# LivGen/LMAT

Measured on AMD Instinct MI355X. Metric: reads/s (150 bp) vs 64 GB k-mer DB, higher is better.
Workload: dtype u64; 1 GPU; 1104000000 x 150 bp reads/GPU vs 64 GiB k-mer hash (6467472668 20-mers, replicated per GPU), run_rl.sh flags -x 0 -j 30 -l 0 -b 1, calls-only; total_reads=1104000000, reads_per_launch=8000000, read_len=150, db_kmers=6467472668, k=20, parallelism=reads sharded x1, DB replicated, genus_block_permille=100, prune_g=0, list_replicas=1, distinct_lists=792576, reads_called=1058323347, read_pool_batches=32

## Files before the change

include/lmat_hip.h:

```cpp
#ifndef LMAT_HIP_H
#define LMAT_HIP_H

#include <stddef.h>
#include <stdint.h>

#ifdef __cplusplus
extern "C" {
#endif

#define LMAT_OK 0
#define LMAT_E_ARG (-1)
#define LMAT_E_IO (-2)
#define LMAT_E_DEVICE (-3)
#define LMAT_E_CAPACITY (-4)
#define LMAT_E_TAXONOMY (-5)
#define LMAT_E_NOMEM (-6)
#define LMAT_E_STATE (-7)
#define LMAT_E_INTERNAL (-8)

typedef struct lmat_ctx lmat_ctx;
typedef struct lmat_reads lmat_reads;
typedef struct lmat_ingest lmat_ingest;
typedef struct lmat_stream lmat_stream;

// ... 219 lines not shown
    uint64_t reads, bases;
    uint64_t windows;
    uint64_t runs;
    uint32_t passes;
    uint32_t prefix_bits;
    float extract_ms, sort_ms, segment_ms, histogram_ms;
} lmat_cov_stats;
int lmat_cov_create(lmat_ctx* ctx, const int* k_sizes, int n_k, lmat_cov** out);
void lmat_cov_destroy(lmat_cov* c);
const char* lmat_cov_error(const lmat_cov* c);
int lmat_cov_set_options(lmat_cov* c, uint64_t device_budget_bytes , int prefix_bits );
int lmat_cov_add_reads(lmat_cov* c, const uint8_t* ascii, const uint64_t* off , uint64_t n_reads, const uint32_t* group);
int lmat_cov_run(lmat_cov* c, lmat_cov_stats* out);
int lmat_cov_summary(lmat_cov* c, int k_index, uint32_t* groups, uint64_t* distinct, uint64_t* total, uint64_t cap, uint64_t* n);
int lmat_cov_histogram(lmat_cov* c, int k_index, uint32_t group, uint64_t* multiplicity, uint64_t* n_kmers, uint64_t cap, uint64_t* n);

int lmat_debug_decide(lmat_ctx* ctx, const uint32_t* tids, const float* scores, const uint64_t* off, const float* stdev,
                      uint64_t n, lmat_read_result* results);
int lmat_debug_decide_counts(lmat_ctx* ctx, const uint32_t* tids, const uint32_t* counts, const uint64_t* off, const uint32_t* cand,
                             uint64_t n, int on_the_wave, lmat_read_result* results);
int lmat_debug_decide_chain(lmat_ctx* ctx, const uint32_t* tids, const uint32_t* counts, const uint64_t* off, const uint32_t* cand,
                            const uint32_t* kept, const uint32_t* eligible, uint64_t n, int with_cands, lmat_read_result* results,
                            uint8_t* took);

int lmat_gather_bench(lmat_ctx* ctx, uint64_t n_probes, uint64_t seed, float* ms, uint64_t* bytes);

int lmat_table_address(int k, uint64_t want_buckets, uint64_t kmer, uint64_t* n_buckets, uint32_t* bucket, uint32_t* tag);
int lmat_table_unaddress(int k, uint64_t want_buckets, uint32_t bucket, uint32_t tag, uint64_t* kmer);

int64_t lmat_format_out(const lmat_ctx* ctx, const lmat_read_result* results, uint64_t n, const lmat_cand* cands,
                        const uint8_t* bases, const uint64_t* off, int prn_read, uint64_t first_index, char* buf,
                        uint64_t cap);

#ifdef __cplusplus
}
#endif
#endif
```

lmat_amd/capi.py:

```python
from __future__ import annotations

import ctypes as C
import os

import numpy as np

_HERE = os.path.dirname(os.path.abspath(__file__))
LIB_PATH = os.environ.get("LMAT_LIB") or os.path.join(_HERE, "liblmat_hip.so")


class LmatError(RuntimeError):
    def __init__(self, code, msg):
        super().__init__(f"lmat error {code}: {msg}")
        self.code = code


class Params(C.Structure):
    _fields_ = [("sdiff", C.c_float), ("hbias", C.c_float), ("min_score", C.c_float), ("min_kmer", C.c_int32),
                ("min_fnd_kmer", C.c_int32), ("prn_all", C.c_int32), ("screen_phix", C.c_int32)]

    @classmethod
    def run_rl(cls, prn_all=1):
        return cls(1.0, 0.0, 0.0, 30, 1, prn_all, 1)

# ... 116 lines not shown
        "lmat_counts_get": (i32, [vp, vp, vp, vp, u32, P(u32), vp]),
        "lmat_gather_bench": (i32, [vp, u64, u64, P(C.c_float), P(u64)]),
        "lmat_stream_create": (i32, [vp, u64, u64, u32, i32, P(vp)]),
        "lmat_stream_acquire": (i32, [vp, P(vp), P(vp)]),
        "lmat_stream_submit": (i32, [vp, u64, u64]),
        "lmat_stream_submit_from": (i32, [vp, vp, vp, u64, u64]),
        "lmat_host_alloc": (i32, [u64, P(vp)]),
        "lmat_host_free": (None, [vp]),
        "lmat_stream_next": (i32, [vp, P(vp), P(vp), P(u64), P(u64), P(u64)]),
        "lmat_stream_release": (i32, [vp]),
        "lmat_stream_destroy": (None, [vp]),
        "lmat_debug_stream_stats": (i32, [vp, vp]),
        "lmat_debug_reads_words": (i32, [vp, vp, u64, u64, vp, vp]),
        "lmat_counts_allreduce": (i32, [P(vp), i32]),
        "lmat_comm_unique_id": (i32, [vp]),
        "lmat_comm_init": (i32, [vp, vp, i32, i32]),
        "lmat_comm_allreduce_counts": (i32, [vp]),
        "lmat_comm_size": (i32, [vp]),
        "lmat_comm_destroy": (None, [vp]),
        "lmat_db_clone": (i32, [vp, vp]),
        "lmat_debug_decide": (i32, [vp, vp, vp, vp, vp, u64, vp]),
        "lmat_debug_decide_counts": (i32, [vp, vp, vp, vp, vp, u64, i32, vp]),
        "lmat_debug_decide_chain": (i32, [vp, vp, vp, vp, vp, vp, vp, u64, i32, vp, vp]),
        "lmat_synth_window": (i32, [vp, u32, u64, P(u64), vp, u32, P(u32)]),
        "lmat_debug_last_counters": (i32, [vp, vp]),
        "lmat_debug_probe_stats": (i32, [vp, vp, u64, vp]),
        "lmat_debug_div_check": (i32, [vp, vp]),
        "lmat_debug_variant_launches": (i32, [vp, vp]),
        "lmat_debug_uniform_launches": (i32, [vp, vp]),
        "lmat_synth_read_windows": (i32, [vp, vp, u32, u64, u64, vp, vp, vp, u32, u32, P(u32), P(u32)]),
        "lmat_table_address": (i32, [i32, u64, u64, P(u64), P(u32), P(u32)]),
        "lmat_format_out": (C.c_int64, [vp, vp, u64, vp, vp, vp, i32, u64, vp, u64]),
        "lmat_build_create": (i32, [vp, i32, cp, P(vp)]),
        "lmat_build_destroy": (None, [vp]),
        "lmat_build_error": (cp, [vp]),
        "lmat_build_set_options": (i32, [vp, u64, i32, u32]),
        "lmat_build_add_fasta": (i32, [vp, cp]),
        "lmat_build_add_sequence": (i32, [vp, u32, vp, u64]),
        "lmat_build_run": (i32, [vp, P(BuildStats)]),
        "lmat_build_write_taxhisto": (i32, [vp, cp]),
        "lmat_build_fetch": (i32, [vp, u64, u64, vp, vp, vp, u64]),
        "lmat_db_build_from_genomes": (i32, [vp, vp, u64]),
        "lmat_build_add_taxhisto": (i32, [vp, cp]),
        "lmat_build_merge_stats": (i32, [vp, P(MergeStats)]),
        "lmat_build_taxid_counts": (i32, [vp, vp, vp, u64, P(u64)]),
        "lmat_cov_create": (i32, [vp, vp, i32, P(vp)]),
# ... 17 lines not shown
        "lmat_table_unaddress": (i32, [i32, u64, u32, u32, P(u64)]),
    }
    for name, (res, args) in sig.items():
        fn = getattr(lib, name)
        fn.restype = res
        fn.argtypes = args
    if path is None:
        _lib = lib
    return lib


EXPORTED = ["lmat_device_count", "lmat_ctx_create", "lmat_ctx_destroy", "lmat_last_error", "lmat_set_params", "lmat_taxonomy_load_files",
            "lmat_db_begin", "lmat_genedb_begin", "lmat_db_add_taxhisto", "lmat_db_finalize", "lmat_db_kmer_length", "lmat_db_size", "lmat_db_list_count", "lmat_db_arena_bytes",
            "lmat_db_set_build_options", "lmat_db_save_image", "lmat_db_load_image", "lmat_ingest_create", "lmat_ingest_idmap_from_tree", "lmat_rand_mode", "lmat_rand_reset", "lmat_rand_label", "lmat_rand_get",
            "lmat_ingest_destroy", "lmat_ingest_error", "lmat_ingest_set_options", "lmat_ingest_add_taxhisto",
            "lmat_ingest_save_image", "lmat_ingest_load_image", "lmat_ingest_size", "lmat_ingest_kmer_length",
            "lmat_ingest_lookup", "lmat_db_from_ingest", "lmat_nullmodel_load", "lmat_nullmodel_clear", "lmat_set_label_modes",
            "lmat_db_table_bytes", "lmat_db_lookup", "lmat_synth_taxonomy", "lmat_synth_db_build", "lmat_synth_db_build2", "lmat_synth_db_build3", "lmat_reads_upload",
            "lmat_reads_synth", "lmat_reads_download_ascii", "lmat_reads_count", "lmat_reads_device_bytes",
            "lmat_reads_free", "lmat_classify", "lmat_classify_async", "lmat_classify_async_cands", "lmat_comm_available", "lmat_sync", "lmat_last_timing", "lmat_results_fetch",
            "lmat_counts_reset", "lmat_counts_layout", "lmat_counts_device_ptr", "lmat_counts_get", "lmat_gather_bench",
            "lmat_table_address", "lmat_format_out", "lmat_stream_create", "lmat_stream_acquire", "lmat_stream_submit", "lmat_stream_submit_from", "lmat_host_alloc", "lmat_host_free",
            "lmat_stream_next", "lmat_stream_release", "lmat_stream_destroy", "lmat_counts_allreduce",
            "lmat_comm_unique_id", "lmat_comm_init", "lmat_comm_allreduce_counts", "lmat_comm_size", "lmat_comm_destroy", "lmat_db_clone", "lmat_debug_decide", "lmat_debug_decide_counts", "lmat_debug_decide_chain", "lmat_synth_window", "lmat_synth_read_windows", "lmat_debug_probe_stats", "lmat_debug_last_counters", "lmat_debug_div_check", "lmat_debug_variant_launches", "lmat_debug_uniform_launches",
            "lmat_build_create", "lmat_build_destroy", "lmat_build_error", "lmat_build_set_options", "lmat_build_add_fasta", "lmat_build_add_sequence",
            "lmat_build_run", "lmat_build_write_taxhisto", "lmat_build_fetch", "lmat_db_build_from_genomes",
            "lmat_build_add_taxhisto", "lmat_build_merge_stats", "lmat_build_taxid_counts",
            "lmat_cov_create", "lmat_cov_destroy", "lmat_cov_error", "lmat_cov_set_options", "lmat_cov_add_reads", "lmat_cov_run",
            "lmat_cov_summary", "lmat_cov_histogram",
            "lmat_export_create", "lmat_export_destroy", "lmat_export_error", "lmat_export_set_options", "lmat_export_run", "lmat_export_fetch",
            "lmat_export_taxid_counts", "lmat_build_add_db", "lmat_table_unaddress",
            "lmat_genebuild_create", "lmat_genedb_build_from_genes",
            "lmat_debug_stream_stats", "lmat_debug_reads_words"]


def _ptr(a):
    return a.ctypes.data_as(C.c_void_p) if a is not None else None


class Reads:
    def __init__(self, eng, handle):
        self.eng, self.h = eng, handle

    def __len__(self):
        return int(self.eng.lib.lmat_reads_count(self.h))

    @property
# ... 699 lines not shown
    def debug_decide_counts(self, tids, counts, off, cand, on_the_wave):
        tids = np.ascontiguousarray(tids, dtype=np.uint32)
        counts = np.ascontiguousarray(counts, dtype=np.uint32)
        off = np.ascontiguousarray(off, dtype=np.uint64)
        cand = np.ascontiguousarray(cand, dtype=np.uint32)
        res = np.zeros(cand.size, dtype=READ_RESULT_DTYPE)
        self._chk(self.lib.lmat_debug_decide_counts(self.ctx, _ptr(tids), _ptr(counts), _ptr(off), _ptr(cand), cand.size, int(on_the_wave), _ptr(res)))
        return res

    def debug_decide_chain(self, tids, counts, off, cand, kept, eligible, with_cands=False):
        tids = np.ascontiguousarray(tids, dtype=np.uint32)
        counts = np.ascontiguousarray(counts, dtype=np.uint32)
        off = np.ascontiguousarray(off, dtype=np.uint64)
        cand = np.ascontiguousarray(cand, dtype=np.uint32)
        kept = np.ascontiguousarray(kept, dtype=np.uint32)
        eligible = np.ascontiguousarray(eligible, dtype=np.uint32)
        assert kept.size == cand.size and eligible.size == cand.size and off.size == cand.size + 1
        res = np.zeros(cand.size, dtype=READ_RESULT_DTYPE)
        took = np.zeros(cand.size, dtype=np.uint8)
        self._chk(self.lib.lmat_debug_decide_chain(self.ctx, _ptr(tids), _ptr(counts), _ptr(off), _ptr(cand), _ptr(kept), _ptr(eligible),
                                                   cand.size, int(with_cands), _ptr(res), _ptr(took)))
        return res, took

    def clone_db_from(self, src: "Engine"):
        self._chk(self.lib.lmat_db_clone(self.ctx, src.ctx))

    def counts(self):
        n, _ = self.counts_layout()
        tid = np.zeros(n, dtype=np.uint32)
        cnt = np.zeros(n, dtype=np.uint64)
        sc = np.zeros(n, dtype=np.float64)
        nz = C.c_uint32(0)
        nm = np.zeros(3, dtype=np.uint64)
        self._chk(self.lib.lmat_counts_get(self.ctx, _ptr(tid), _ptr(cnt), _ptr(sc), n, C.byref(nz), _ptr(nm)))
        k = int(nz.value)
        return {int(t): (int(c), float(s)) for t, c, s in zip(tid[:k], cnt[:k], sc[:k])}, [int(x) for x in nm]
```

lmat_amd/csrc/kernels.hip:

```cpp
#include <hip/hip_runtime.h>
#include <atomic>
#include <type_traits>
#include "kernels.hpp"

#ifndef LMAT_ABLATE
#define LMAT_ABLATE 0
#endif
#define STOP_AT(n, v) do { if (LMAT_ABLATE && A.prm.stop_after == (n)) { if (lane == 0) { emit(250, (v)); } return; } } while (0)
#ifndef LMAT_CLOSURE_FAST
#define LMAT_CLOSURE_FAST 1
#endif
#ifndef LMAT_LDS_SHIFT
#define LMAT_LDS_SHIFT 0
#endif

namespace lmat {

#define WSYNC()                                              \
    do {                                                     \
        __builtin_amdgcn_fence(__ATOMIC_SEQ_CST, "wavefront"); \
        __builtin_amdgcn_wave_barrier();                     \
    } while (0)

template <bool GMEM>
// ... 939 lines not shown
    }
    if (bad) atomicAdd(out + 2, (unsigned long long)bad);
    atomicAdd(out + 3, 64ull);
}
typedef const ClassifyArgs __attribute__((address_space(4))) CArgsK4;
typedef float f32x4 __attribute__((ext_vector_type(4)));
__device__ __forceinline__ uint64_t bal(bool b) { return __builtin_amdgcn_ballot_w64(b); }
__device__ __forceinline__ void k4_wave_record(CArgsK4* Ap, int lane, GAS uint64_t* out, const lmat_read_result& res, uint32_t call_idx) {
    if (lane == 0) {
        GAS unsigned long long* tally_count = (GAS unsigned long long*)Ap->counts;
        GAS double* tally_score = (GAS double*)(tally_count + Ap->tb.n_ids);
        GAS unsigned long long* tally_nomatch = (GAS unsigned long long*)(tally_score + Ap->tb.n_ids);
        store_result(out, res);
        if (res.status != LMAT_ST_PHIX && res.match_type == LMAT_MT_NOMATCH) {
            G_ADD(&tally_nomatch[1], 1ull);
        } else if (res.call_score >= Ap->prm.min_score) {
            G_ADD(&tally_count[call_idx], 1ull);
            G_ADD(&tally_score[call_idx], (double)res.call_score);
        } else if (res.call_score < Ap->prm.min_score) {
            G_ADD(&tally_nomatch[2], 1ull);
        }
    }
}
__device__ __forceinline__ bool k4_wave_chain(CArgsK4* Ap, int lane, uint32_t nT, uint32_t cand, const u32x4 fz, uint32_t my_cnt,
                                              uint32_t my_id, uint32_t dep, uint32_t fl, uint32_t chain, uint32_t* xch, GAS uint64_t* out,
                                              int valid_kmers, uint32_t len, int bin_sel) {
    const uint32_t sx0 = chain & 63u, nK = (chain >> 8) & 0x7Fu;
    if (nK - 1u >= nT - 1u || sx0 >= nK) return false;
    const uint64_t am = below_mask_1_64((int)nT), KEPT = below_mask_1_64((int)nK), CH = am & ~KEPT, OTH = KEPT & ~(1ull << sx0);
    const uint32_t ti = fz.z & 0xFFFFu, oi = fz.z >> 16;
    const uint32_t c0 = rl(my_cnt, (int)sx0), riv = rl(fz.z, (int)sx0);
    const uint32_t rt = riv & 0xFFFFu, ro = riv >> 16;
    const uint32_t badfl = (uint32_t)kFlagPlasmid | (Ap->prm.screen_phix ? (uint32_t)kFlagPhiX : 0u);
    if ((~bal(my_cnt < c0) & OTH) | (~bal(my_cnt == c0) & CH)) return false;
    if ((~(bal(oi < rt) | bal(ro < ti)) & OTH) | (~(bal(ti < rt) & bal(ro <= oi)) & CH)) return false;
    if (!(bal(dep == 0u) & CH) || bal((fl & badfl) != 0)) return false;
    float* xs = (float*)xch;
    float* xv = (float*)(xch + 256);
    const float sc = div_small_ints((float)my_cnt, (float)cand);
    xs[lane] = sc;
    WSYNC();
    float log_sum = 0.0f;
    for (uint32_t t = 0; t < nT; t += 4) {
        const u32x4 q = *(const u32x4*)((const uint32_t*)xs + t);
        log_sum += __uint_as_float(q.x); log_sum += __uint_as_float(q.y); log_sum += __uint_as_float(q.z); log_sum += __uint_as_float(q.w);
    }
    const uint32_t pos_sig_hits = (uint32_t)popc64(bal(my_cnt > 0));
    const uint32_t use_sig_hits = pos_sig_hits > 3 ? pos_sig_hits : nT;
    const float log_avg = div_small_ints(log_sum, (float)use_sig_hits);
    const float dv = log_avg - sc;
    xv[lane] = (uint32_t)lane < nT && (pos_sig_hits > 3 ? my_cnt > 0 : true) ? dv * dv : 0.0f;
    WSYNC();
    float log_std = 0.0f;
    for (uint32_t t = 0; t < nT; t += 4) {
        const f32x4 q = *(const f32x4*)(xv + t);
        log_std += q.x; log_std += q.y; log_std += q.z; log_std += q.w;
    }
    const float stdev1 = use_sig_hits > 1 ? sqrtf(div_small_ints(log_std, (float)(use_sig_hits - 1))) : 0.0f;
    const float diff_thresh = stdev1 * Ap->prm.sdiff;
    const float s0 = __uint_as_float(rl(__float_as_uint(sc), (int)sx0));
    const float d = s0 - sc;
    uint64_t close = bal(d <= diff_thresh) & OTH;
    uint8_t match = LMAT_MT_DIRECT;
    uint32_t call_tid = rl(my_id, (int)sx0);
    float call_score = s0;
    if (close) {
        uint64_t good = CH;
        do {
            const uint32_t ivj = rl(fz.z, __builtin_ctzll(close));
            close &= close - 1;
            good &= bal(ti < (ivj & 0xFFFFu)) & bal((ivj >> 16) <= oi);
        } while (close && good);
        if (!good) {
            match = LMAT_MT_LCA_ERROR; call_tid = 0; call_score = 0;
        } else {
            const uint32_t k = wave_max_u32(lane_bit(good) ? (ti << 6) | (uint32_t)lane : 0u);
            match = LMAT_MT_MULTI; call_tid = rl(my_id, (int)(k & 63u));
        }
    }
    lmat_read_result res;
    res.status = LMAT_ST_CALL; res.match_type = match; res.cand_kmer_cnt = (uint16_t)cand; res.valid_kmers = valid_kmers;
    res.read_len = (int)len; res.log_avg = log_avg; res.stdev = stdev1; res.cand_off = 0; res.n_cand = 0; res.bin_sel = bin_sel;
    res.call_tid = call_tid ? ((const GAS uint32_t*)Ap->tb.tid32)[call_tid] : 0u;
    res.call_score = call_score;
    k4_wave_record(Ap, lane, out, res, call_tid);
    return true;
}
template <int THM, bool PLAIN = false>
__device__ __forceinline__ bool k4_wave(CArgsK4* Ap, int lane, uint32_t nT, uint32_t cand, const u32x4 fz, uint32_t my_cnt,
                                        uint32_t my_id, const unsigned int* hent, uint32_t* xch, GAS uint64_t* out,
                                        int valid_kmers, uint32_t len, int bin_sel, uint32_t chain = 0, uint32_t* took_chain = nullptr) {
    const float hbias = PLAIN ? 0.0f : Ap->prm.hbias, sdiff = Ap->prm.sdiff;
    const int screen_phix = Ap->prm.screen_phix;
    if (!PLAIN && !(Ap->prm.k4_static & 1)) return false;
    const int stop = LMAT_ABLATE ? Ap->prm.stop_after : 0;
    auto placeholder = [&]() {
        if (lane == 0) {
            uint32_t z = 0;
            asm volatile("" : "+v"(z));
            out[0] = (uint64_t)(z + ((uint32_t)LMAT_ST_SILENT | ((uint32_t)LMAT_MT_NOMATCH << 8) | (cand << 16))) | ((uint64_t)(uint32_t)valid_kmers << 32);
            out[1] = (uint64_t)len | ((uint64_t)z << 32);
            out[2] = (uint64_t)z | ((uint64_t)z << 32);
            out[3] = (uint64_t)z | ((uint64_t)z << 32);
            out[4] = (uint64_t)z | ((uint64_t)(uint32_t)bin_sel << 32);
        }
        return true;
    };
    if (stop == 30 || (stop == 34 && nT <= 16)) return placeholder();
    if (cand - 1u > 998u || nT - 1u > 63u) return false;
    const bool act = (uint32_t)lane < nT;
    const uint32_t dep = act ? (fz.w & 0xFFFFu) : 0u, fl = act ? (fz.w >> 16) : 0u;
    if (bal(my_cnt > cand) | bal(dep > 0x7FFFu) | (hbias != 0.0f ? bal((fl & kFlagHuman) != 0) : 0ull)) return false;
    if (LMAT_ABLATE && lane == 0) { G_ADD((GAS uint32_t*)Ap->cursor + kCurChainSeen, 1u); if (chain) G_ADD((GAS uint32_t*)Ap->cursor + kCurChainLone, 1u); }
    if (chain && (PLAIN || (Ap->prm.k4_static & 4)) &&
        k4_wave_chain(Ap, lane, nT, cand, fz, my_cnt, my_id, dep, fl, chain, xch, out, valid_kmers, len, bin_sel)) {
        if (LMAT_ABLATE && lane == 0) G_ADD((GAS uint32_t*)Ap->cursor + kCurChainTaken, 1u);
        if (took_chain) *took_chain = 1u;
        return true;
    }
    float* xs = (float*)xch;
    uint32_t* xk = xch + 64;
    uint32_t* xx = xch + 128;
    float* xv = (float*)(xch + 256);
    uint32_t* xp = xch + 320;
    const float fcand = (float)cand;
    const float sc = div_small_ints((float)my_cnt, fcand);
    xs[lane] = sc;
    uint32_t e = act ? (((my_cnt << 15) | dep) << 6) | (uint32_t)lane : 0xFFFFFFFFu;
    if (nT > 16) {
        int lg = 0;
        for (uint32_t t = nT; t > 1; t >>= 1) ++lg;
        uint32_t st0 = 0, st1 = 0, st2 = 0;
        int sp = 0, first = 0, last = (int)nT, depth = 2 * lg;
        bool busy = true;
        while (busy) {
            if (last - first <= 16) {
                if (sp > 0) {
                    --sp;
                    const uint32_t top = sp == 0 ? st0 : (sp == 1 ? st1 : st2);
                    first = (int)(top & 0xFFu); last = (int)((top >> 8) & 0xFFu); depth = (int)(top >> 16);
                } else busy = false;
// ... 1794 lines not shown
            if (act) {
                pe = g_paths8[poff_i + rel];
                pf = ((const GAS uint8_t*)tb.paths_fl)[poff_i + rel];
                a = (uint32_t)(pe & 0xFFFFu);
                h = tid_find_or_claim(hent, THM, a);
                atomicMin(&hent[h], a | ((0x8000u | (uint32_t)lane) << 16));
            }
            WSYNC();
            const uint64_t nm_ = __ballot(i < W) & __ballot((hent[h] >> 16) == (0x8000u | (uint32_t)lane));
            const uint32_t newcnt = popc64(nm_);
            if (nT + newcnt > (uint32_t)T) { overflow = true; break; }
            if (lane_bit(nm_)) {
                const uint32_t s = nT + prefix_count(nm_);
                hent[h] = a | (s << 16);
                reg[s] = (uint16_t)a;
                anc_zw[s] = u32x2{(uint32_t)(pe >> 32), ((uint32_t)(pe >> 16) & 0xFFFFu) | (pf << 16)};
            }
            nT += newcnt;
            WSYNC();
        }
        STOP_AT(45, nT);
        if (!overflow && (uint32_t)lane >= nT_p1 && (uint32_t)lane < nT) { const u32x2 zw = anc_zw[lane]; fz = u32x4{0u, 0u, zw.x, zw.y}; }
        const bool lone = one && !overflow && W > 0 && nT - nT_p1 == W && cand == nuniq;
        if (lone) {
            const uint32_t c0 = cnt[sx0];
            if ((uint32_t)lane >= nT_p1 && (uint32_t)lane < nT) cnt[lane] = (uint16_t)c0;
            chain = 0x10000u | (nT_p1 << 8) | (uint32_t)sx0;
            WSYNC();
        } else if (!overflow && W > 0) {
            const bool sl_act = (uint32_t)lane < nT;
            uint32_t tin_s = 0xFFFF, tout_s = 0;
            if (sl_act) { tin_s = fz.z & 0xFFFFu; tout_s = fz.z >> 16; }
            uint32_t anc_lo = 0, anc_hi = 0;
            uint64_t todo = todo0;
            while (todo) {
                const int sx = __builtin_ctzll(todo);
                todo &= todo - 1;
                const uint32_t tin_x = (uint32_t)__builtin_amdgcn_readlane((int)tin_s, sx);
                const uint32_t tout_x = (uint32_t)__builtin_amdgcn_readlane((int)tout_s, sx);
                const uint64_t am = __ballot(tin_s < tin_x) & __ballot(tout_x <= tout_s);
                uint32_t m0_keep;
                asm("s_mov_b32 %2, m0\n\ts_mov_b32 m0, %4\n\tv_writelane_b32 %0, %3, m0\n\tv_writelane_b32 %1, %5, m0\n\ts_mov_b32 m0, %2"
                    : "+v"(anc_lo), "+v"(anc_hi), "=&s"(m0_keep) : "s"((uint32_t)am), "s"(sx), "s"((uint32_t)(am >> 32)));
            }
            unsigned int* memw = (unsigned int*)el_t;
            unsigned int* hitw = (unsigned int*)el_off;
            static_assert(2 * E >= 512 && sizeof(*el_t) == 2 && sizeof(*el_off) == 2, "64 mask pairs fit each of the two dead arrays");
            *(u32x2*)(memw + 2 * lane) = u32x2{0u, 0u};
            *(u32x2*)(hitw + 2 * lane) = u32x2{0u, 0u};
            const bool wide_t = nT > 32u;
// ... 782 lines not shown
    if (small_stream != stream && small_stream != stream3) hipStreamWaitEvent(small_stream, forked, 0);
    launch_k4_lds<kK4SmallT>(a, a.count, small_stream);
}
void launch_k4_end(const ClassifyArgs& a, hipStream_t join_stream, hipStream_t stream2, hipStream_t stream3, hipStream_t small_stream,
                   hipEvent_t joined2, hipEvent_t joined3, hipEvent_t joined_small, hipEvent_t done) {
    if (stream2 != join_stream) { hipEventRecord(joined2, stream2); hipStreamWaitEvent(join_stream, joined2, 0); }
    if (stream3 != join_stream) { hipEventRecord(joined3, stream3); hipStreamWaitEvent(join_stream, joined3, 0); }
    if (small_stream != join_stream && small_stream != stream3 && small_stream != stream2) {
        hipEventRecord(joined_small, small_stream);
        hipStreamWaitEvent(join_stream, joined_small, 0);
    }
    ClassifyArgs b = a;
    b.k4_slot = kCurK4Bail;
    if (a.nm.active) k4_kernel<true, kK4T, 64><<<dim3(64), dim3(64), 0, join_stream>>>(b);
    else k4_kernel<false, kK4T, 64><<<dim3(64), dim3(64), 0, join_stream>>>(b);
    hipEventRecord(done, join_stream);
}

static int k4_static_of(const ClassifyArgs& a) {
    const int stop = a.prm.stop_after;
    const bool base = !a.nm.active && a.tb.depth_consistent && !(a.cands && !a.prm.prn_all);
    const bool wave = base && (stop == 0 || (stop >= 30 && stop <= 34));
    const bool rows = base && a.prm.k4_row && stop == 0;
    const bool chain = wave && stop == 0 && !a.cands && a.prm.k4_chain;
    return (wave ? 1 : 0) | (rows ? 2 : 0) | (chain ? 4 : 0);
}
static bool plain_launch(const ClassifyArgs& a, int k4_static) {
    static const bool on = !LMAT_ABLATE && (!getenv("LMAT_PLAIN") || atoi(getenv("LMAT_PLAIN")) != 0);
    return on && a.tb.k == 20 && a.tb.cpt.nb && a.tb.cpt.m == 17 && a.tb.cpt.lowbits == 2 && !a.tb.wide && !a.nm.active && !a.rand_max &&
           !a.gene_mode && !a.prm.permissive && a.prm.stop_after == 0 && k4_static == 5 && !a.cands && a.prm.hbias == 0.0f &&
           a.p_min == 0 && a.p_max == 0xFFFFFFFFu && !a.index && !a.count_ptr && a.tail_lpr == 4;
}
static bool uniform_launch(const ClassifyArgs& a) {
    static const bool on = !getenv("LMAT_UNIFORM") || atoi(getenv("LMAT_UNIFORM")) != 0;
    return on && a.uniform;
}
static std::atomic<unsigned long long> g_variant_launches[64][3];
void classify_variant_launches(int device, uint64_t out[2]) {
    out[0] = out[1] = 0;
    if (device < 0 || device >= 64) return;
    out[0] = g_variant_launches[device][0].load();
    out[1] = g_variant_launches[device][1].load();
}
uint64_t classify_uniform_launches(int device) { return device < 0 || device >= 64 ? 0 : g_variant_launches[device][2].load(); }
template <int U, int T, int E, bool INK4, bool PERM, bool CPT, bool WIDE = false, bool PLAIN = false, bool UNI = false>
static void launch_classify_t(const ClassifyArgs& a_in, hipStream_t stream) {
    using L = WL<U, T, E, INK4, CPT, WIDE>;
    ClassifyArgs a = a_in;
    a.prm.k4_static = k4_static_of(a);
    constexpr bool kPlainClass = U == 160 && T == 64 && E == kFastE && !INK4 && !PERM && CPT && !WIDE;
    if constexpr (kPlainClass && !PLAIN && !LMAT_ABLATE) {
        if (plain_launch(a, a.prm.k4_static)) {
            if (uniform_launch(a)) launch_classify_t<U, T, E, INK4, PERM, CPT, WIDE, true, true>(a_in, stream);
// ... 23 lines not shown
    int grid = 256 * (per_cu < 1 ? 1 : (per_cu > 32 ? 32 : per_cu)) * (gmult > 0 ? gmult : 32);
    if (!a.count_ptr && (uint64_t)grid > a.count) grid = (int)a.count;
    if (a.count_ptr && INK4 && grid > 256 * (per_cu < 2 ? 2 : per_cu)) grid = 256 * (per_cu < 2 ? 2 : per_cu);
    if (grid < 1) grid = 1;
    classify_kernel<U, T, E, INK4, PERM, CPT, WIDE, PLAIN, UNI><<<dim3(grid), dim3(64), lds_bytes, stream>>>(a);
}

void launch_k4_debug(const ClassifyArgs& a, const uint32_t* idx, const float* scores, const uint64_t* off, const float* stdevs, uint64_t n,
                     hipStream_t stream) {
    if (!n) return;
    k4_debug_kernel<<<dim3((unsigned)((n + 63) / 64)), dim3(64), 0, stream>>>(a, idx, scores, off, stdevs, n);
}

void launch_k4_debug_counts(const ClassifyArgs& a, const uint32_t* idx, const uint32_t* cnts, const uint64_t* off, const uint32_t* cands, uint64_t n,
                            bool on_the_wave, hipStream_t stream, const uint32_t* shape, uint8_t* took) {
    if (!n) return;
    if (on_the_wave) {
        const uint64_t g = n < 256 * 32 ? n : 256 * 32;
        ClassifyArgs b = a;
        b.prm.k4_static = k4_static_of(b);
        k4_wave_debug_kernel<<<dim3((unsigned)g), dim3(64), 0, stream>>>(b, idx, cnts, off, cands, n, shape, took);
    } else k4_debug_counts_kernel<<<dim3((unsigned)((n + 63) / 64)), dim3(64), 0, stream>>>(a, idx, cnts, off, cands, n);
}

void launch_tail(const ClassifyArgs& a, hipStream_t stream) {
    if (!a.tail_lpr || !a.count || a.count_ptr) return;
    const uint64_t lanes = a.count * a.tail_lpr;
    const dim3 grid((unsigned)((lanes + 255) / 256));
    if (a.tail_lpr == 4) tail_kernel<4><<<grid, dim3(256), 0, stream>>>(a);
    else if (a.tail_lpr == 8) tail_kernel<8><<<grid, dim3(256), 0, stream>>>(a);
    else tail_kernel<16><<<grid, dim3(256), 0, stream>>>(a);
}

int classify_max_read_len() { return kGmemU + 19; }
size_t classify_gmem_scratch_bytes() { return (size_t)kGmemGrid * WL<kGmemU, 4096, 16384, true, false, true>::BYTES; }

#define LC(U, T, E, K)                                                                                                   \
    (a.tb.cpt.nb ? (a.prm.permissive ? launch_classify_t<U, T, E, K, true, true>(a, stream) : launch_classify_t<U, T, E, K, false, true>(a, stream)) \
                 : (a.prm.permissive ? launch_classify_t<U, T, E, K, true, false>(a, stream) : launch_classify_t<U, T, E, K, false, false>(a, stream)))
#define LCW(U, T, E) (a.prm.permissive ? launch_classify_t<U, T, E, true, true, true, true>(a, stream) : launch_classify_t<U, T, E, true, false, true, true>(a, stream))
bool launch_classify(const ClassifyArgs& a, uint32_t max_read_len, int tcap_class, hipStream_t stream) {
    const int k = a.tb.k;
    const uint32_t P = max_read_len >= (uint32_t)k ? max_read_len - k + 1 : 0;
    if (a.tb.wide) {
        if (!a.tb.cpt.nb) return false;
        if (tcap_class == 4) { if (P > 512) return false; LCW(512, 128, 512); }
// ... 96 lines not shown
```

lmat_amd/csrc/kernels.hpp:

```cpp
#pragma once
#include "lmat_internal.hpp"

namespace lmat {

struct ClassifyArgs {
    DeviceTables tb;
    KernelParams prm;
    const uint32_t* words;
    const uint64_t* rec_off;
    const uint32_t* index;
    uint32_t p_min = 0, p_max = 0xFFFFFFFFu;
    uint64_t first, count;
    uint64_t result_base;
    lmat_read_result* results;
    lmat_cand* cands;
    uint64_t cand_cap;
    uint32_t* cursor;
    uint32_t cand_chunk = 0;
    uint32_t cand_sub_mask = 0;
    uint32_t* err;
    void* counts;
    uint32_t phix_call_idx;
    uint32_t* ovf_list;
    uint32_t ovf_slot;
// ... 18 lines not shown
    uint32_t uniform = 0;
};

static const int kK4T = 64;
static const int kK4RecWords = 2 + kK4T;

static const int kCandSubs = 1024;
static const int kCursorWords = 16;
static const size_t kCursorBytes = kCursorWords * 4 + (size_t)kCandSubs * 64;
enum CursorWord {
    kCurCand = 0,
    kCurOvfFast = 2,
    kCurOvfE512 = 3,
    kCurOvfMid = 10,
    kCurOvfLarge = 7,
    kCurK4Small = 4,
    kCurK4Large = 5,
    kCurK4Mid = 8,
    kCurK4Row = 9,
    kCurK4Bail = 6,
    kCurChainSeen = 11,
    kCurChainLone = 12,
    kCurChainTaken = 13,
    kCurBatchErr = 15,
};

enum { kErrTidOverflow = 1, kErrReadTooLong = 2, kErrCandOverflow = 4, kErrLineageTrunc = 8, kErrNoNullModel = 16 };

void launch_fill_offsets(uint64_t* off, uint64_t* rec_off, uint64_t n, uint32_t len, hipStream_t stream);
void launch_pack_reads(const uint8_t* bases, const uint64_t* off, const uint64_t* rec_off, uint32_t* words, uint64_t n,
                       hipStream_t stream);
void launch_insert_pairs(const DeviceTables& tb, const uint64_t* kmers, const uint32_t* payload, uint64_t n,
                         uint32_t* fail, hipStream_t stream);
void launch_synth_db(const DeviceTables& tb, const SynthGeo& g, int k, const uint16_t* strain_idx, const uint32_t* list_payload,
                     uint64_t g_off, uint32_t rep, uint32_t rep_stride, uint32_t* fail, unsigned long long* inserted, hipStream_t stream);
void launch_table_count(const DeviceTables& tb, unsigned long long* out, hipStream_t stream);
void launch_synth_reads(uint32_t* words, const uint64_t* rec_off, const uint32_t* lengths, uint32_t n_lengths, uint64_t n,
                        uint64_t seed, const SynthGeo& g, hipStream_t stream);
void launch_lookup(const DeviceTables& tb, const uint64_t* kmers, uint64_t n, uint32_t* counts, uint32_t* tids,
                   uint32_t stride, hipStream_t stream);
void launch_div_check(unsigned long long* out2, hipStream_t stream);
void launch_probe_stats(const DeviceTables& tb, const uint64_t* kmers, uint64_t n, unsigned long long* out, hipStream_t stream);
void launch_tail(const ClassifyArgs& a, hipStream_t stream);
bool launch_classify(const ClassifyArgs& a, uint32_t max_read_len, int tcap_class, hipStream_t stream);
void launch_k4_begin(const ClassifyArgs& a, hipStream_t stream, hipStream_t stream2, hipStream_t stream3, hipStream_t small_stream,
                     hipEvent_t forked);
// ... 22 lines not shown
```

lmat_amd/csrc/lmat_api.cpp:

```cpp
#include <hip/hip_runtime.h>
#include <algorithm>
#include <cmath>
#include <cstdio>
#include <cstring>
#include <chrono>
#include <string>
#include <thread>
#include <atomic>
#include <fcntl.h>
#include <unistd.h>
#include "kernels.hpp"
#include "outfmt.hpp"

using namespace lmat;

#define HIPCHK(ctx, call)                                                                          \
    do {                                                                                           \
        hipError_t e__ = (call);                                                                   \
        if (e__ != hipSuccess)                                                                     \
            return set_err(ctx, LMAT_E_DEVICE, std::string(#call) + ": " + hipGetErrorString(e__)); \
    } while (0)

template <class T>
static int dev_upload(lmat_ctx* c, T** dst, const std::vector<T>& src) {
// ... 45 lines not shown
        if ((rc = dev_upload(c, &c->dev.facts16, f16))) return rc;
    }
    c->dev.n_ids = T.n + 1;
    c->dev.depth_consistent = 1;
    for (uint32_t i = 1; i <= T.n; ++i)
        if (T.path_len[i] && T.fdepth[i] <= T.fdepth[T.paths[T.path_off[i]]]) { c->dev.depth_consistent = 0; break; }
    if (c->d_counts) { hipFree(c->d_counts); c->d_counts = nullptr; }
    c->counts_bytes = (uint64_t)c->dev.n_ids * 16 + 24;
    HIPCHK(c, hipMalloc(&c->d_counts, c->counts_bytes));
    HIPCHK(c, hipMemset(c->d_counts, 0, c->counts_bytes));
    return LMAT_OK;
}
}

static KernelParams kparams(const lmat_params& p) {
    KernelParams k;
    k.sdiff = p.sdiff; k.hbias = p.hbias; k.min_score = p.min_score;
    k.min_kmer = p.min_kmer; k.min_fnd_kmer = p.min_fnd_kmer; k.prn_all = p.prn_all; k.screen_phix = p.screen_phix;
    k.permissive = 0;
    const char* sa = getenv("LMAT_STOP_AFTER");
    k.stop_after = sa ? atoi(sa) : 0;
    if (const char* w = getenv("LMAT_K4_WAVE")) if (!k.stop_after && atoi(w) == 0) k.stop_after = 20;
    k.k4_row = getenv("LMAT_K4_ROW") && atoi(getenv("LMAT_K4_ROW")) != 0;
    k.k4_chain = !(getenv("LMAT_K4_CHAIN") && atoi(getenv("LMAT_K4_CHAIN")) == 0);
    k.k4_static = 0;
    return k;
}

extern "C" {

static void sb_free(lmat_ctx* c);
static int sb_begin(lmat_ctx* c, uint64_t n_kmers, uint64_t table_bytes, int k);
static int sb_push(lmat_ctx* c, Ingest& B);

int lmat_device_count(void) {
    int n = 0;
    return hipGetDeviceCount(&n) == hipSuccess ? n : 0;
}

int lmat_ctx_create(int device, const lmat_params* params, lmat_ctx** out) {
    if (!out) return LMAT_E_ARG;
    *out = nullptr;
    int ndev = 0;
    if (hipGetDeviceCount(&ndev) != hipSuccess || ndev <= 0 || device < 0 || device >= ndev) return LMAT_E_DEVICE;
    if (hipSetDevice(device) != hipSuccess) return LMAT_E_DEVICE;
    lmat_ctx* c = new lmat_ctx();
    c->device = device;
// ... 1733 lines not shown
        a.cand_cap = total;
        a.prm.prn_all = 1;
    }
    launch_k4_debug_counts(a, d_idx.as<uint32_t>(), d_cn.as<uint32_t>(), d_off.as<uint64_t>(), d_cd.as<uint32_t>(), n, on_the_wave != 0, c->stream,
                           shape ? d_shape.as<uint32_t>() : nullptr, took ? d_took.as<uint8_t>() : nullptr);
    if (took) HIPCHK(c, hipMemcpyAsync(took, d_took.p, n, hipMemcpyDeviceToHost, c->stream));
    return debug_fetch(c, d_res, n, results);
}
int lmat_debug_decide_counts(lmat_ctx* c, const uint32_t* tids, const uint32_t* counts, const uint64_t* off, const uint32_t* cand, uint64_t n,
                             int on_the_wave, lmat_read_result* results) {
    if (!c || !tids || !counts || !off || !cand || !results) return LMAT_E_ARG;
    return debug_decide_counts(c, tids, counts, off, cand, n, on_the_wave, nullptr, 0, results, nullptr);
}
int lmat_debug_decide_chain(lmat_ctx* c, const uint32_t* tids, const uint32_t* counts, const uint64_t* off, const uint32_t* cand,
                            const uint32_t* kept, const uint32_t* eligible, uint64_t n, int with_cands, lmat_read_result* results, uint8_t* took) {
    if (!c || !tids || !counts || !off || !cand || !kept || !eligible || !results || !took) return LMAT_E_ARG;
    std::vector<uint32_t> shape(n);
    for (uint64_t i = 0; i < n; ++i) {
        if (kept[i] > 64u || (kept[i] && eligible[i] >= kept[i])) return set_err(c, LMAT_E_ARG, "kept slots above 64, or an eligible slot that is not among them");
        shape[i] = kept[i] ? (0x10000u | (kept[i] << 8) | eligible[i]) : 0u;
    }
    return debug_decide_counts(c, tids, counts, off, cand, n, 1, &shape, with_cands, results, took);
}

int lmat_debug_last_counters(lmat_ctx* c, uint32_t* out16) {
    if (!c || !out16) return LMAT_E_ARG;
    hipSetDevice(c->device);
    HIPCHK(c, hipMemcpy(out16, c->set().cursor.p, kCursorWords * 4, hipMemcpyDeviceToHost));
    return LMAT_OK;
}

int lmat_debug_variant_launches(lmat_ctx* c, uint64_t* out2) {
    if (!c || !out2) return LMAT_E_ARG;
    classify_variant_launches(c->device, out2);
    return LMAT_OK;
}
int lmat_debug_uniform_launches(lmat_ctx* c, uint64_t* out) {
    if (!c || !out) return LMAT_E_ARG;
    *out = classify_uniform_launches(c->device);
    return LMAT_OK;
}

int lmat_last_timing(const lmat_ctx* c, float* classify_ms, float* decide_ms, uint64_t* launches) {
    if (!c) return LMAT_E_ARG;
    if (classify_ms) *classify_ms = c->last_classify_ms;
    if (decide_ms) *decide_ms = c->last_decide_ms;
// ... 447 lines not shown
```

Baseline: 400.7 million reads/s.

## Add closed-form path fast path to wave decision for single-path candidate sets

```diff
diff --git a/include/lmat_hip.h b/include/lmat_hip.h
--- a/include/lmat_hip.h
+++ b/include/lmat_hip.h
@@ -265,6 +265,8 @@
 int lmat_debug_decide_chain(lmat_ctx* ctx, const uint32_t* tids, const uint32_t* counts, const uint64_t* off, const uint32_t* cand,
                             const uint32_t* kept, const uint32_t* eligible, uint64_t n, int with_cands, lmat_read_result* results,
                             uint8_t* took);
+int lmat_debug_decide_shape(lmat_ctx* ctx, const uint32_t* tids, const uint32_t* counts, const uint64_t* off, const uint32_t* cand,
+                            const uint32_t* shape, uint64_t n, int with_cands, lmat_read_result* results, uint8_t* took);
 
 int lmat_gather_bench(lmat_ctx* ctx, uint64_t n_probes, uint64_t seed, float* ms, uint64_t* bytes);
 
diff --git a/lmat_amd/capi.py b/lmat_amd/capi.py
--- a/lmat_amd/capi.py
+++ b/lmat_amd/capi.py
@@ -162,6 +162,7 @@
         "lmat_debug_decide": (i32, [vp, vp, vp, vp, vp, u64, vp]),
         "lmat_debug_decide_counts": (i32, [vp, vp, vp, vp, vp, u64, i32, vp]),
         "lmat_debug_decide_chain": (i32, [vp, vp, vp, vp, vp, vp, vp, u64, i32, vp, vp]),
+        "lmat_debug_decide_shape": (i32, [vp, vp, vp, vp, vp, vp, u64, i32, vp, vp]),
         "lmat_synth_window": (i32, [vp, u32, u64, P(u64), vp, u32, P(u32)]),
         "lmat_debug_last_counters": (i32, [vp, vp]),
         "lmat_debug_probe_stats": (i32, [vp, vp, u64, vp]),
@@ -225,7 +226,7 @@
             "lmat_counts_reset", "lmat_counts_layout", "lmat_counts_device_ptr", "lmat_counts_get", "lmat_gather_bench",
             "lmat_table_address", "lmat_format_out", "lmat_stream_create", "lmat_stream_acquire", "lmat_stream_submit", "lmat_stream_submit_from", "lmat_host_alloc", "lmat_host_free",
             "lmat_stream_next", "lmat_stream_release", "lmat_stream_destroy", "lmat_counts_allreduce",
-            "lmat_comm_unique_id", "lmat_comm_init", "lmat_comm_allreduce_counts", "lmat_comm_size", "lmat_comm_destroy", "lmat_db_clone", "lmat_debug_decide", "lmat_debug_decide_counts", "lmat_debug_decide_chain", "lmat_synth_window", "lmat_synth_read_windows", "lmat_debug_probe_stats", "lmat_debug_last_counters", "lmat_debug_div_check", "lmat_debug_variant_launches", "lmat_debug_uniform_launches",
+            "lmat_comm_unique_id", "lmat_comm_init", "lmat_comm_allreduce_counts", "lmat_comm_size", "lmat_comm_destroy", "lmat_db_clone", "lmat_debug_decide", "lmat_debug_decide_counts", "lmat_debug_decide_chain", "lmat_debug_decide_shape", "lmat_synth_window", "lmat_synth_read_windows", "lmat_debug_probe_stats", "lmat_debug_last_counters", "lmat_debug_div_check", "lmat_debug_variant_launches", "lmat_debug_uniform_launches",
             "lmat_build_create", "lmat_build_destroy", "lmat_build_error", "lmat_build_set_options", "lmat_build_add_fasta", "lmat_build_add_sequence",
             "lmat_build_run", "lmat_build_write_taxhisto", "lmat_build_fetch", "lmat_db_build_from_genomes",
             "lmat_build_add_taxhisto", "lmat_build_merge_stats", "lmat_build_taxid_counts",
@@ -971,6 +972,19 @@
                                                    cand.size, int(with_cands), _ptr(res), _ptr(took)))
         return res, took
 
+    def debug_decide_shape(self, tids, counts, off, cand, shape, with_cands=False):
+        tids = np.ascontiguousarray(tids, dtype=np.uint32)
+        counts = np.ascontiguousarray(counts, dtype=np.uint32)
+        off = np.ascontiguousarray(off, dtype=np.uint64)
+        cand = np.ascontiguousarray(cand, dtype=np.uint32)
+        shape = np.ascontiguousarray(shape, dtype=np.uint32)
+        assert shape.size == cand.size and off.size == cand.size + 1
+        res = np.zeros(cand.size, dtype=READ_RESULT_DTYPE)
+        took = np.zeros(cand.size, dtype=np.uint8)
+        self._chk(self.lib.lmat_debug_decide_shape(self.ctx, _ptr(tids), _ptr(counts), _ptr(off), _ptr(cand), _ptr(shape), cand.size,
+                                                   int(with_cands), _ptr(res), _ptr(took)))
+        return res, took
+
     def clone_db_from(self, src: "Engine"):
         self._chk(self.lib.lmat_db_clone(self.ctx, src.ctx))
 
diff --git a/lmat_amd/csrc/kernels.hip b/lmat_amd/csrc/kernels.hip
--- a/lmat_amd/csrc/kernels.hip
+++ b/lmat_amd/csrc/kernels.hip
@@ -985,6 +985,42 @@
         }
     }
 }
+__device__ __forceinline__ float k4_wave_stats(int lane, uint32_t nT, uint32_t cand, uint32_t my_cnt, uint32_t* xch, float& log_avg, float& stdev1) {
+    float* xs = (float*)xch;
+    float* xv = (float*)(xch + 256);
+    const float sc = div_small_ints((float)my_cnt, (float)cand);
+    xs[lane] = sc;
+    WSYNC();
+    float log_sum = 0.0f;
+#pragma nounroll
+    for (uint32_t t = 0; t < nT; t += 4) {
+        const u32x4 q = *(const u32x4*)((const uint32_t*)xs + t);
+        log_sum += __uint_as_float(q.x); log_sum += __uint_as_float(q.y); log_sum += __uint_as_float(q.z); log_sum += __uint_as_float(q.w);
+    }
+    const uint32_t pos_sig_hits = (uint32_t)popc64(bal(my_cnt > 0));
+    const uint32_t use_sig_hits = pos_sig_hits > 3 ? pos_sig_hits : nT;
+    log_avg = div_small_ints(log_sum, (float)use_sig_hits);
+    const float dv = log_avg - sc;
+    xv[lane] = (uint32_t)lane < nT && (pos_sig_hits > 3 ? my_cnt > 0 : true) ? dv * dv : 0.0f;
+    WSYNC();
+    float log_std = 0.0f;
+#pragma nounroll
+    for (uint32_t t = 0; t < nT; t += 4) {
+        const f32x4 q = *(const f32x4*)(xv + t);
+        log_std += q.x; log_std += q.y; log_std += q.z; log_std += q.w;
+    }
+    stdev1 = use_sig_hits > 1 ? sqrtf(div_small_ints(log_std, (float)(use_sig_hits - 1))) : 0.0f;
+    return sc;
+}
+__device__ __forceinline__ void k4_wave_closed_record(CArgsK4* Ap, int lane, GAS uint64_t* out, uint8_t match, uint32_t call_tid, float call_score,
+                                                      uint32_t cand, float log_avg, float stdev1, int valid_kmers, uint32_t len, int bin_sel) {
+    lmat_read_result res;
+    res.status = LMAT_ST_CALL; res.match_type = match; res.cand_kmer_cnt = (uint16_t)cand; res.valid_kmers = valid_kmers;
+    res.read_len = (int)len; res.log_avg = log_avg; res.stdev = stdev1; res.cand_off = 0; res.n_cand = 0; res.bin_sel = bin_sel;
+    res.call_tid = call_tid ? ((const GAS uint32_t*)Ap->tb.tid32)[call_tid] : 0u;
+    res.call_score = call_score;
+    k4_wave_record(Ap, lane, out, res, call_tid);
+}
 __device__ __forceinline__ bool k4_wave_chain(CArgsK4* Ap, int lane, uint32_t nT, uint32_t cand, const u32x4 fz, uint32_t my_cnt,
                                               uint32_t my_id, uint32_t dep, uint32_t fl, uint32_t chain, uint32_t* xch, GAS uint64_t* out,
                                               int valid_kmers, uint32_t len, int bin_sel) {
@@ -998,28 +1034,8 @@
     if ((~bal(my_cnt < c0) & OTH) | (~bal(my_cnt == c0) & CH)) return false;
     if ((~(bal(oi < rt) | bal(ro < ti)) & OTH) | (~(bal(ti < rt) & bal(ro <= oi)) & CH)) return false;
     if (!(bal(dep == 0u) & CH) || bal((fl & badfl) != 0)) return false;
-    float* xs = (float*)xch;
-    float* xv = (float*)(xch + 256);
-    const float sc = div_small_ints((float)my_cnt, (float)cand);
-    xs[lane] = sc;
-    WSYNC();
-    float log_sum = 0.0f;
-    for (uint32_t t = 0; t < nT; t += 4) {
-        const u32x4 q = *(const u32x4*)((const uint32_t*)xs + t);
-        log_sum += __uint_as_float(q.x); log_sum += __uint_as_float(q.y); log_sum += __uint_as_float(q.z); log_sum += __uint_as_float(q.w);
-    }
-    const uint32_t pos_sig_hits = (uint32_t)popc64(bal(my_cnt > 0));
-    const uint32_t use_sig_hits = pos_sig_hits > 3 ? pos_sig_hits : nT;
-    const float log_avg = div_small_ints(log_sum, (float)use_sig_hits);
-    const float dv = log_avg - sc;
-    xv[lane] = (uint32_t)lane < nT && (pos_sig_hits > 3 ? my_cnt > 0 : true) ? dv * dv : 0.0f;
-    WSYNC();
-    float log_std = 0.0f;
-    for (uint32_t t = 0; t < nT; t += 4) {
-        const f32x4 q = *(const f32x4*)(xv + t);
-        log_std += q.x; log_std += q.y; log_std += q.z; log_std += q.w;
-    }
-    const float stdev1 = use_sig_hits > 1 ? sqrtf(div_small_ints(log_std, (float)(use_sig_hits - 1))) : 0.0f;
+    float log_avg, stdev1;
+    const float sc = k4_wave_stats(lane, nT, cand, my_cnt, xch, log_avg, stdev1);
     const float diff_thresh = stdev1 * Ap->prm.sdiff;
     const float s0 = __uint_as_float(rl(__float_as_uint(sc), (int)sx0));
     const float d = s0 - sc;
@@ -1041,12 +1057,64 @@
             match = LMAT_MT_MULTI; call_tid = rl(my_id, (int)(k & 63u));
         }
     }
-    lmat_read_result res;
-    res.status = LMAT_ST_CALL; res.match_type = match; res.cand_kmer_cnt = (uint16_t)cand; res.valid_kmers = valid_kmers;
-    res.read_len = (int)len; res.log_avg = log_avg; res.stdev = stdev1; res.cand_off = 0; res.n_cand = 0; res.bin_sel = bin_sel;
-    res.call_tid = call_tid ? ((const GAS uint32_t*)Ap->tb.tid32)[call_tid] : 0u;
-    res.call_score = call_score;
-    k4_wave_record(Ap, lane, out, res, call_tid);
+    k4_wave_closed_record(Ap, lane, out, match, call_tid, call_score, cand, log_avg, stdev1, valid_kmers, len, bin_sel);
+    return true;
+}
+#if LMAT_ABLATE
+__device__ uint32_t g_path_why[16];
+#define PATH_WHY(i) do { if (lane == 0) atomicAdd(&g_path_why[i], 1u); } while (0)
+#else
+#define PATH_WHY(i) ((void)0)
+#endif
+__device__ __forceinline__ bool k4_wave_path(CArgsK4* Ap, int lane, uint32_t nT, uint32_t cand, const u32x4 fz, uint32_t my_cnt,
+                                             uint32_t my_id, uint32_t dep, uint32_t fl, uint32_t chain, uint32_t* xch, GAS uint64_t* out,
+                                             int valid_kmers, uint32_t len, int bin_sel) {
+    const uint32_t nK = (chain >> 8) & 0x7Fu;
+    PATH_WHY(0);
+    if (nK - 1u >= nT) { PATH_WHY(2); return false; }
+    const uint64_t am = below_mask_1_64((int)nT);
+    const uint32_t kv = wave_max_u32((uint32_t)lane < nK ? (my_cnt << 6) | (uint32_t)lane : 0u);
+    const uint32_t v = kv & 63u, c0 = kv >> 6;
+    const uint32_t ti = fz.z & 0xFFFFu, oi = fz.z >> 16;
+    const uint32_t riv = rl(fz.z, (int)v);
+    const uint32_t rt = riv & 0xFFFFu, ro = riv >> 16;
+    const uint64_t CH = bal(ti < rt) & bal(ro <= oi) & am, PATH = CH | (1ull << v), OTH = am & ~PATH;
+    if (!CH) { PATH_WHY(3); return false; }
+    if (~bal(my_cnt < c0) & OTH) { PATH_WHY(4); return false; }
+    if (~bal(my_cnt >= c0) & CH) { PATH_WHY(5); return false; }
+    if (~(bal(oi < rt) | bal(ro < ti)) & OTH) { PATH_WHY(6); return false; }
+    if (!(bal(dep == 0u) & CH)) { PATH_WHY(7); return false; }
+    const uint32_t badfl = (uint32_t)kFlagPlasmid | (Ap->prm.screen_phix ? (uint32_t)kFlagPhiX : 0u);
+    if (bal((fl & badfl) != 0)) { PATH_WHY(8); return false; }
+    float log_avg, stdev1;
+    const float sc = k4_wave_stats(lane, nT, cand, my_cnt, xch, log_avg, stdev1);
+    const float diff_thresh = stdev1 * Ap->prm.sdiff;
+    const float s0 = __uint_as_float(rl(__float_as_uint(sc), (int)v));
+    uint64_t close = bal(s0 - sc <= diff_thresh) & OTH;
+    uint8_t match = LMAT_MT_DIRECT;
+    uint32_t call_tid = rl(my_id, (int)v);
+    float call_score = s0;
+    if (close) {
+        uint64_t good = CH;
+        do {
+            const int j = __builtin_ctzll(close);
+            close &= close - 1;
+            const uint32_t ivj = rl(fz.z, j);
+            const float sj = __uint_as_float(rl(__float_as_uint(sc), j));
+            const uint64_t anc = bal(ti < (ivj & 0xFFFFu)) & bal((ivj >> 16) <= oi);
+            if (bal(sc - sj > diff_thresh) & PATH & ~anc) { PATH_WHY(9); return false; }
+            good &= anc;
+        } while (close);
+        if (!good) {
+            match = LMAT_MT_LCA_ERROR; call_tid = 0; call_score = 0;
+        } else {
+            const uint32_t k = wave_max_u32(lane_bit(good) ? (ti << 6) | (uint32_t)lane : 0u);
+            match = LMAT_MT_MULTI; call_tid = rl(my_id, (int)(k & 63u));
+            call_score = __uint_as_float(wave_max_u32(lane_bit(PATH) && ti >= (k >> 6) ? __float_as_uint(sc) : 0u));
+        }
+    }
+    PATH_WHY(1);
+    k4_wave_closed_record(Ap, lane, out, match, call_tid, call_score, cand, log_avg, stdev1, valid_kmers, len, bin_sel);
     return true;
 }
 template <int THM, bool PLAIN = false>
@@ -1074,12 +1142,20 @@
     const bool act = (uint32_t)lane < nT;
     const uint32_t dep = act ? (fz.w & 0xFFFFu) : 0u, fl = act ? (fz.w >> 16) : 0u;
     if (bal(my_cnt > cand) | bal(dep > 0x7FFFu) | (hbias != 0.0f ? bal((fl & kFlagHuman) != 0) : 0ull)) return false;
-    if (LMAT_ABLATE && lane == 0) { G_ADD((GAS uint32_t*)Ap->cursor + kCurChainSeen, 1u); if (chain) G_ADD((GAS uint32_t*)Ap->cursor + kCurChainLone, 1u); }
-    if (chain && (PLAIN || (Ap->prm.k4_static & 4)) &&
+    if (LMAT_ABLATE && lane == 0) { G_ADD((GAS uint32_t*)Ap->cursor + kCurChainSeen, 1u); if (chain & 0x10000u) G_ADD((GAS uint32_t*)Ap->cursor + kCurChainLone, 1u); }
+    if ((chain & 0x10000u) && (PLAIN || (Ap->prm.k4_static & 4)) &&
         k4_wave_chain(Ap, lane, nT, cand, fz, my_cnt, my_id, dep, fl, chain, xch, out, valid_kmers, len, bin_sel)) {
         if (LMAT_ABLATE && lane == 0) G_ADD((GAS uint32_t*)Ap->cursor + kCurChainTaken, 1u);
         if (took_chain) *took_chain = 1u;
         return true;
+    }
+    if ((chain & 0x20000u) && (PLAIN || (Ap->prm.k4_static & 8))) {
+        if (LMAT_ABLATE && lane == 0) G_ADD((GAS uint32_t*)Ap->cursor + kCurPathSeen, 1u);
+        if (k4_wave_path(Ap, lane, nT, cand, fz, my_cnt, my_id, dep, fl, chain, xch, out, valid_kmers, len, bin_sel)) {
+            if (LMAT_ABLATE && lane == 0) G_ADD((GAS uint32_t*)Ap->cursor + kCurPathTaken, 1u);
+            if (took_chain) *took_chain = 2u;
+            return true;
+        }
     }
     float* xs = (float*)xch;
     uint32_t* xk = xch + 64;
@@ -2920,10 +2996,11 @@
         STOP_AT(45, nT);
         if (!overflow && (uint32_t)lane >= nT_p1 && (uint32_t)lane < nT) { const u32x2 zw = anc_zw[lane]; fz = u32x4{0u, 0u, zw.x, zw.y}; }
         const bool lone = one && !overflow && W > 0 && nT - nT_p1 == W && cand == nuniq;
+        if (!overflow) chain = 0x20000u | (nT_p1 << 8);
         if (lone) {
             const uint32_t c0 = cnt[sx0];
             if ((uint32_t)lane >= nT_p1 && (uint32_t)lane < nT) cnt[lane] = (uint16_t)c0;
-            chain = 0x10000u | (nT_p1 << 8) | (uint32_t)sx0;
+            chain |= 0x10000u | (uint32_t)sx0;
             WSYNC();
         } else if (!overflow && W > 0) {
             const bool sl_act = (uint32_t)lane < nT;
@@ -3752,13 +3829,13 @@
     const bool base = !a.nm.active && a.tb.depth_consistent && !(a.cands && !a.prm.prn_all);
     const bool wave = base && (stop == 0 || (stop >= 30 && stop <= 34));
     const bool rows = base && a.prm.k4_row && stop == 0;
-    const bool chain = wave && stop == 0 && !a.cands && a.prm.k4_chain;
-    return (wave ? 1 : 0) | (rows ? 2 : 0) | (chain ? 4 : 0);
+    const bool closed = wave && stop == 0 && !a.cands;
+    return (wave ? 1 : 0) | (rows ? 2 : 0) | (closed && (a.prm.k4_chain & 1) ? 4 : 0) | (closed && (a.prm.k4_chain & 2) ? 8 : 0);
 }
 static bool plain_launch(const ClassifyArgs& a, int k4_static) {
     static const bool on = !LMAT_ABLATE && (!getenv("LMAT_PLAIN") || atoi(getenv("LMAT_PLAIN")) != 0);
     return on && a.tb.k == 20 && a.tb.cpt.nb && a.tb.cpt.m == 17 && a.tb.cpt.lowbits == 2 && !a.tb.wide && !a.nm.active && !a.rand_max &&
-           !a.gene_mode && !a.prm.permissive && a.prm.stop_after == 0 && k4_static == 5 && !a.cands && a.prm.hbias == 0.0f &&
+           !a.gene_mode && !a.prm.permissive && a.prm.stop_after == 0 && k4_static == 13 && !a.cands && a.prm.hbias == 0.0f &&
            a.p_min == 0 && a.p_max == 0xFFFFFFFFu && !a.index && !a.count_ptr && a.tail_lpr == 4;
 }
 static bool uniform_launch(const ClassifyArgs& a) {
@@ -3828,6 +3905,17 @@
         k4_wave_debug_kernel<<<dim3((unsigned)g), dim3(64), 0, stream>>>(b, idx, cnts, off, cands, n, shape, took);
     } else k4_debug_counts_kernel<<<dim3((unsigned)((n + 63) / 64)), dim3(64), 0, stream>>>(a, idx, cnts, off, cands, n);
 }
+
+#if LMAT_ABLATE
+}
+extern "C" int lmat_ablate_path_why(uint32_t* out16, int reset) {
+    if (hipDeviceSynchronize() != hipSuccess) return -1;
+    if (out16 && hipMemcpyFromSymbol(out16, HIP_SYMBOL(lmat::g_path_why), 64) != hipSuccess) return -1;
+    if (reset) { const uint32_t z[16] = {0}; if (hipMemcpyToSymbol(HIP_SYMBOL(lmat::g_path_why), z, 64) != hipSuccess) return -1; }
+    return 0;
+}
+namespace lmat {
+#endif
 
 void launch_tail(const ClassifyArgs& a, hipStream_t stream) {
     if (!a.tail_lpr || !a.count || a.count_ptr) return;
diff --git a/lmat_amd/csrc/kernels.hpp b/lmat_amd/csrc/kernels.hpp
--- a/lmat_amd/csrc/kernels.hpp
+++ b/lmat_amd/csrc/kernels.hpp
@@ -64,6 +64,8 @@
     kCurChainSeen = 11,
     kCurChainLone = 12,
     kCurChainTaken = 13,
+    kCurPathSeen = 14,
+    kCurPathTaken = 1,
     kCurBatchErr = 15,
 };
 
diff --git a/lmat_amd/csrc/lmat_api.cpp b/lmat_amd/csrc/lmat_api.cpp
--- a/lmat_amd/csrc/lmat_api.cpp
+++ b/lmat_amd/csrc/lmat_api.cpp
@@ -91,7 +91,8 @@
     k.stop_after = sa ? atoi(sa) : 0;
     if (const char* w = getenv("LMAT_K4_WAVE")) if (!k.stop_after && atoi(w) == 0) k.stop_after = 20;
     k.k4_row = getenv("LMAT_K4_ROW") && atoi(getenv("LMAT_K4_ROW")) != 0;
-    k.k4_chain = !(getenv("LMAT_K4_CHAIN") && atoi(getenv("LMAT_K4_CHAIN")) == 0);
+    k.k4_chain = !(getenv("LMAT_K4_CHAIN") && atoi(getenv("LMAT_K4_CHAIN")) == 0) ? 1 : 0;
+    if (!(getenv("LMAT_K4_PATH") && atoi(getenv("LMAT_K4_PATH")) == 0)) k.k4_chain |= 2;
     k.k4_static = 0;
     return k;
 }
@@ -1871,6 +1872,17 @@
     }
     return debug_decide_counts(c, tids, counts, off, cand, n, 1, &shape, with_cands, results, took);
 }
+int lmat_debug_decide_shape(lmat_ctx* c, const uint32_t* tids, const uint32_t* counts, const uint64_t* off, const uint32_t* cand,
+                            const uint32_t* shape, uint64_t n, int with_cands, lmat_read_result* results, uint8_t* took) {
+    if (!c || !tids || !counts || !off || !cand || !shape || !results || !took) return LMAT_E_ARG;
+    std::vector<uint32_t> sh(shape, shape + n);
+    for (uint64_t i = 0; i < n; ++i) {
+        const uint32_t kept = (sh[i] >> 8) & 0xFFu, el = sh[i] & 0xFFu;
+        if ((sh[i] & ~0x3FFFFu) || kept > 64u || ((sh[i] & 0x10000u) && el >= kept) || (!(sh[i] & 0x10000u) && el) || (!(sh[i] & 0x30000u) && sh[i]))
+            return set_err(c, LMAT_E_ARG, "a shape word with kept slots above 64, an eligible slot that is not among them, or bits without their flag");
+    }
+    return debug_decide_counts(c, tids, counts, off, cand, n, 1, &sh, with_cands, results, took);
+}
 
 int lmat_debug_last_counters(lmat_ctx* c, uint32_t* out16) {
     if (!c || !out16) return LMAT_E_ARG;
```

Result: faster. 425.6 million reads/s, median of 6 (+6.2%).
